# dioph/periodicity

Hardware: AMD Instinct MI355X
Metric: Lomb-Scargle Gpair/s (sample x freq), fp64, N=1e5 x 1e6 per GPU (higher is better)
Workload: dtype f64

## Files before the change

periodicity_amd/_cabi.py:

```python
import ctypes as C
import os
import threading

import numpy as np

_LIB_NAME = "libperiodicity_hip.so"
_lib = None
_lock = threading.Lock()

c_double_p = C.POINTER(C.c_double)
c_int64_p = C.POINTER(C.c_int64)

STATUS_EXC = {-1: ValueError, -2: RuntimeError, -3: RuntimeError, -4: RuntimeError,
              -5: MemoryError}

_VP, _I, _L, _D = C.c_void_p, C.c_int, C.c_int64, C.c_double
PROTOTYPES = {
    "pdc_last_error": (C.c_char_p, []),
    "pdc_version": (_I, []),
    "pdc_device_count": (_I, [C.POINTER(_I)]),
    "pdc_device_info": (_I, [_I, C.c_char_p, _I, C.POINTER(_I), c_int64_p, C.POINTER(_I)]),
    "pdc_release": (_I, []),
    "pdc_alloc_counts": (_I, [c_int64_p, c_int64_p]),
    "pdc_malloc": (_I, [_I, _L, C.POINTER(_VP)]),
# ... 366 lines not shown


def wwz_tile_bins():
    return int(lib().pdc_wwz_tile_bins())


def wwz_work_bytes(n, nf, ntau):
    return int(lib().pdc_wwz_work_bytes(int(n), int(nf), int(ntau)))


def wwz_last_dispatch():
    k, rows, launches = C.c_int(0), C.c_int(0), C.c_int64(0)
    check(lib().pdc_wwz_last_dispatch(C.byref(k), C.byref(rows), C.byref(launches)))
    return k.value, rows.value, launches.value


def bls_scan(t, y, dy, periods, n_bins, len_min, len_max, min_points=5, dips_only=False, slices=0, device=None):
    t, y, periods = _f64(t, "t"), _f64(y, "y"), _f64(periods, "periods")
    dy = None if dy is None else _f64(dy, "dy")
    if y.size != t.size or (dy is not None and dy.size != t.size):
        raise ValueError("Input arrays have incompatible lengths.")
    power, depth = np.empty(periods.size, dtype=np.float64), np.empty(periods.size, dtype=np.float64)
    start, box = np.empty(periods.size, dtype=np.int32), np.empty(periods.size, dtype=np.int32)
    dev = default_device() if device is None else device
    check(lib().pdc_bls_scan(_ptr(t), _ptr(y), _ptr(dy), t.size, _ptr(periods), periods.size, int(n_bins), int(len_min),
                             int(len_max), int(min_points), int(bool(dips_only)), int(slices), _ptr(power), _ptr(depth),
                             _ptr(start), _ptr(box), dev))
    return power, depth, start, box


def gls_scan_batch(t, y, dy, offsets, f0, delta, nf, fit_mean=True, psd=False, shared_t=False,
                   want_power=True, want_peaks=False, j_begin=0, device=None, devices=None):
    t, y = _f64(t, "t"), _f64(y, "y")
    dy = None if dy is None else _f64(dy, "dy")
    offsets = np.ascontiguousarray(offsets, dtype=np.int64)
    nb = offsets.size - 1
    if nb < 1 or offsets[-1] != y.size or (dy is not None and dy.size != y.size):
        raise ValueError("Input arrays have incompatible lengths.")
    if (shared_t and t.size != offsets[1]) or (not shared_t and t.size != y.size):
        raise ValueError("Input arrays have incompatible lengths.")
    power = np.empty((nb, nf), dtype=np.float64) if want_power else None
    amax = np.empty(nb, dtype=np.float64) if want_peaks else None
    argmax = np.empty(nb, dtype=np.int64) if want_peaks else None
    if devices is not None and len(devices) > 1:
        if j_begin:
            raise ValueError("a batch sharded over devices scans the whole grid (j_begin must be 0)")
        devs = np.ascontiguousarray(devices, dtype=np.int32)
        check(lib().pdc_gls_scan_batch_multi(_ptr(t), _ptr(y), _ptr(dy), _ptr(offsets), nb, int(shared_t),
                                             f0, delta, nf, int(bool(fit_mean)), int(bool(psd)),
                                             _ptr(power), _ptr(amax), _ptr(argmax), _ptr(devs), devs.size))
        return power, amax, argmax
    device = pick_device(device, devices)
    dev = default_device() if device is None else device
    check(lib().pdc_gls_scan_batch(_ptr(t), _ptr(y), _ptr(dy), _ptr(offsets), nb, int(shared_t),
                                   f0, delta, j_begin, nf, int(bool(fit_mean)), int(bool(psd)),
                                   _ptr(power), _ptr(amax), _ptr(argmax), dev))
    return power, amax, argmax


def gls_bootstrap(t, y, dy, picks, f0, delta, nf, fit_mean=True, psd=False, method="direct", device=None,
                  devices=None):
    t, y = _f64(t, "t"), _f64(y, "y")
    dy = None if dy is None else _f64(dy, "dy")
    picks = np.ascontiguousarray(picks, dtype=np.int32)
    if y.size != t.size or (dy is not None and dy.size != t.size):
        raise ValueError("Input arrays have incompatible lengths.")
    if picks.ndim != 2 or (picks.shape[0] and picks.shape[1] != t.size):
        raise ValueError("picks must be [n_bootstraps][n_samples]")
    nb = picks.shape[0]
    amax = np.empty(nb, dtype=np.float64)
    argmax = np.empty(nb, dtype=np.int64)
    if devices is not None and len(devices) > 0:
        devs = np.ascontiguousarray(devices, dtype=np.int32)
    else:
        devs = np.array([default_device() if device is None else device], dtype=np.int32)
    check(lib().pdc_gls_bootstrap(_ptr(t), _ptr(y), _ptr(dy), t.size, _ptr(picks), nb, float(f0), float(delta),
                                  int(nf), int(bool(fit_mean)), int(bool(psd)), 1 if method == "fft" else 0,
                                  _ptr(amax), _ptr(argmax), _ptr(devs), devs.size))
    return amax, argmax


GLS_ROUTES = ("none", "general", "parts", "balanced", "shared", "shared2")
_GLS_DISPATCH_FIELDS = ("route", "K", "S", "tiles", "parts", "parts_by_xcd", "bal_slots", "wide_prep", "bpad", "groups",
                        "z_len", "bal_chunks", "lead_swap")


def gls_last_dispatch():
    out = (C.c_int64 * len(_GLS_DISPATCH_FIELDS))()
    check(lib().pdc_test_gls_last_dispatch(out))
    rec = dict(zip(_GLS_DISPATCH_FIELDS, (int(v) for v in out)))
    rec["route"] = GLS_ROUTES[rec["route"]]
    return rec


def gls_last_pair():
    out = (C.c_int64 * 2)()
    check(lib().pdc_test_gls_last_pair(out))
    return bool(out[0]), int(out[1])


def gls_scan_multi(t, y, dy, f0, delta, nf, fit_mean=True, psd=False, devices=(0,)):
    t, y = _f64(t, "t"), _f64(y, "y")
    dy = None if dy is None else _f64(dy, "dy")
    if y.size != t.size or (dy is not None and dy.size != t.size):
        raise ValueError("Input arrays have incompatible lengths.")
    devs = np.ascontiguousarray(devices, dtype=np.int32)
    out = np.empty(nf, dtype=np.float64)
    check(lib().pdc_gls_scan_multi(_ptr(t), _ptr(y), _ptr(dy), t.size, f0, delta, nf,
                                   int(bool(fit_mean)), int(bool(psd)), _ptr(out), _ptr(devs),
                                   devs.size))
    return out


class GlsPlan:

    def __init__(self, devices, n_max, nf_max, loopback_slots=None):
        devs = np.ascontiguousarray(devices, dtype=np.int32)
        self._plan = C.c_void_p()
        if loopback_slots is not None:
            if devs.size != 1:
                raise ValueError("a loopback plan lives on one device")
            self.devices = [int(devs[0])] * int(loopback_slots)
            check(lib().pdc_gls_plan_create_loopback(int(devs[0]), int(loopback_slots), int(n_max),
                                                     int(nf_max), C.byref(self._plan)))
        else:
            self.devices = [int(d) for d in devs]
            check(lib().pdc_gls_plan_create(_ptr(devs), devs.size, int(n_max), int(nf_max),
                                            C.byref(self._plan)))
        self.nf = 0

    def info(self):
        n, r, x = C.c_int(0), C.c_int(0), C.c_int(0)
        check(lib().pdc_gls_plan_info(self._plan, C.byref(n), C.byref(r), C.byref(x)))
        buf = C.create_string_buffer(512)
        check(lib().pdc_gls_plan_init_error(self._plan, buf, 512))
        return {"n_slots": n.value, "rccl_ranks": r.value, "exchange": ("none", "rccl", "copy")[x.value],
                "init_error": buf.value.decode() or None}

    def upload(self, t, y, dy=None):
        t, y = _f64(t, "t"), _f64(y, "y")
        dy = None if dy is None else _f64(dy, "dy")
        if y.size != t.size or (dy is not None and dy.size != t.size):
            raise ValueError("Input arrays have incompatible lengths.")
        check(lib().pdc_gls_plan_upload(self._plan, _ptr(t), _ptr(y), _ptr(dy), t.size))

    def scan(self, f0, delta, nf, fit_mean=True, psd=False):
        check(lib().pdc_gls_plan_scan(self._plan, float(f0), float(delta), int(nf),
                                      int(bool(fit_mean)), int(bool(psd))))
        self.nf = int(nf)

    def wait(self):
        check(lib().pdc_gls_plan_wait(self._plan))

    def download(self, which=0):
        out = np.empty(self.nf, dtype=np.float64)
        check(lib().pdc_gls_plan_download(self._plan, _ptr(out), self.nf, int(which)))
        return out

    def kernel_ms(self):
        ms = C.c_float()
        check(lib().pdc_gls_plan_kernel_ms(self._plan, C.byref(ms)))
        return ms.value

    def slot_ms(self):
        ms = (C.c_float * len(self.devices))()
        check(lib().pdc_gls_plan_slot_ms(self._plan, ms, len(self.devices)))
        return [float(v) for v in ms]
# ... 385 lines not shown
```

periodicity_amd/csrc/gls.hip:

```cpp
#include "pdc_internal.h"
#include "gls_epilogue.h"
#include "gls_sums.h"

#include <cstdlib>

using namespace pdc;

namespace {

constexpr int kBlock = 256;
constexpr int kPrepBlock = 1024;

enum Mode { MODE_FIT_MEAN = 0, MODE_NO_MEAN = 1, MODE_RAW = 2, MODE_TREND = 3 };
constexpr bool mode_fits_mean(int m) { return m == MODE_FIT_MEAN; }
constexpr bool mode_sums_w(int m) { return m == MODE_FIT_MEAN || m == MODE_TREND; }

struct TrendScalars {
    double W;
    double yy, y1, ty, tt, t1;
    double shift;
    double inv_span;
    double prec_a, prec_alpha, prec_beta;
    double log_const;
};

struct GlsArgs {
    const double *rec;
    const int64_t *offsets;
    const double *scal;
    int64_t n_total, n_curves, tiles;
    double f0, delta;
    int64_t j_begin, nf;
    int psd;
    int lead_swap = 0;
    double *power;
    double *raw_s;
    double *raw_c;
    double *blk_max;
    int64_t *blk_arg;
    int64_t z_len = 0;
    int parts = 1, parts_by_xcd = 0;
    double *partial = nullptr;
    int64_t bal_slots = 0, bal_units = 0, bal_chunks = 0, bal_tile_freqs = 0;
    TrendScalars trend = {};
    const double *pair_tab = nullptr;
};

__device__ __forceinline__ int64_t bal_slot_of(const GlsArgs &a, int64_t x) {
    int64_t s = x * a.bal_slots / a.bal_units;
    while ((s + 1) * a.bal_units / a.bal_slots <= x) ++s;
    while (s * a.bal_units / a.bal_slots > x) --s;
    return s;
}

struct PrepArgs {
    const double *t, *y, *dy;
    const int64_t *offsets;
    int64_t n_total;
    int shared_t, fit_mean, raw;
    double delta;
    double *rec, *scal;
    double *rw = nullptr;
    double *tp = nullptr;
    int64_t bpad = 0;
    const int32_t *picks = nullptr;
};

__global__ __launch_bounds__(kPrepBlock) void gls_prep_kernel(PrepArgs a) {
    __shared__ double red[kPrepBlock / 64];
    const int tid = threadIdx.x;
    const int64_t off = a.offsets ? a.offsets[blockIdx.x] : 0;
    const int64_t n = a.offsets ? a.offsets[blockIdx.x + 1] - off : a.n_total;
    const double *t = a.shared_t ? a.t : a.t + off;
    const int32_t *pk = a.picks ? a.picks + off : nullptr;
    const double *y = pk ? a.y : a.y + off;
    const double *dy = a.dy ? (pk ? a.dy : a.dy + off) : nullptr;
    auto at = [pk](int64_t i) -> int64_t { return pk ? (int64_t)pk[i] : i; };
    double *rec = a.rec + off * 6;
    const double t0 = n > 0 ? t[0] : 0.0;

    double W = 1.0, ybar = 0.0;
    if (!a.raw) {
        double acc = 0.0;
        for (int64_t i = tid; i < n; i += kPrepBlock) {
            const double e = dy ? dy[at(i)] : 1.0;
            acc += 1.0 / (e * e);
        }
        W = block_sum<kPrepBlock>(acc, red);
        if (a.fit_mean) {
            acc = 0.0;
            for (int64_t i = tid; i < n; i += kPrepBlock) {
                const double e = dy ? dy[at(i)] : 1.0;
                acc += (1.0 / (e * e)) / W * y[at(i)];
            }
            ybar = block_sum<kPrepBlock>(acc, red);
        }
    }
    double yy = 0.0, wsum = 0.0;
    if (a.rw) {
        for (int64_t i = tid; i < n; i += kPrepBlock) {
            const double e = dy ? dy[at(i)] : 1.0;
            const double w = (1.0 / (e * e)) / W;
            const double yc = y[at(i)] - ybar;
            const double wy = w * yc;
            yy += wy * yc;
            wsum += w;
            if (dy) reinterpret_cast<double2 *>(a.rw)[i * a.bpad + blockIdx.x] = make_double2(wy, w);
            else a.rw[i * a.bpad + blockIdx.x] = wy;
            if (blockIdx.x == 0) a.tp[i] = t[i] - t0;
        }
    } else
    for (int64_t i = tid; i < n; i += kPrepBlock) {
        const double tp = t[i] - t0;
        double w, wy;
        if (a.raw) {
            w = y[at(i)];
            wy = w;
// ... 41 lines not shown
    for (int64_t i = (int64_t)blockIdx.x * kBlock + threadIdx.x; i < a.p.n_total;
         i += (int64_t)gridDim.x * kBlock) {
        const double wr = inv_var(a.p.dy, i);
        sw += wr;
        swy += wr * a.p.y[i];
    }
    sw = block_sum<kBlock>(sw, red);
    swy = block_sum<kBlock>(swy, red);
    if (threadIdx.x == 0) {
        a.part[blockIdx.x] = sw;
        a.part[kPrepParts + blockIdx.x] = swy;
    }
}

__device__ __forceinline__ double fold_partials(const double *p, int count, double *red) {
    double v = 0.0;
    for (int i = threadIdx.x; i < count; i += kBlock) v += p[i];
    return block_sum<kBlock>(v, red);
}

__global__ __launch_bounds__(kBlock) void gls_prep_wide_b(WidePrepArgs a) {
    __shared__ double red[kBlock / 64];
    const double W = fold_partials(a.part, a.nparts, red);
    const double ybar = a.p.fit_mean ? fold_partials(a.part + kPrepParts, a.nparts, red) / W : 0.0;
    const double t0 = a.p.t[0];
    double yy = 0.0, wsum = 0.0;
    for (int64_t i = (int64_t)blockIdx.x * kBlock + threadIdx.x; i < a.p.n_total;
         i += (int64_t)gridDim.x * kBlock) {
        const double tp = a.p.t[i] - t0;
        const double w = inv_var(a.p.dy, i) / W;
        const double yc = a.p.y[i] - ybar;
        const double wy = w * yc;
        yy += wy * yc;
        wsum += w;
        double sd, cd;
        sincos_cycles(frac_product(a.p.delta, tp), sd, cd);
        const double rw = sqrt(w);
        double2 *r = reinterpret_cast<double2 *>(a.p.rec + i * 6);
        r[0] = make_double2(rw * yc, rw);
        r[1] = make_double2(cd, sd);
        r[2] = make_double2(cd + cd, tp);
    }
    yy = block_sum<kBlock>(yy, red);
    wsum = block_sum<kBlock>(wsum, red);
    if (threadIdx.x == 0) {
        a.part[2 * kPrepParts + blockIdx.x] = yy;
        a.part[3 * kPrepParts + blockIdx.x] = wsum;
    }
}

__global__ __launch_bounds__(kBlock) void gls_prep_wide_c(WidePrepArgs a) {
    __shared__ double red[kBlock / 64];
    const double W = fold_partials(a.part, a.nparts, red);
    const double yy = fold_partials(a.part + 2 * kPrepParts, a.nparts, red);
    const double wsum = fold_partials(a.part + 3 * kPrepParts, a.nparts, red);
    if (threadIdx.x == 0) {
        a.p.scal[0] = yy;
        a.p.scal[1] = wsum;
        a.p.scal[2] = W;
        a.p.scal[3] = a.p.t[0];
    }
}

constexpr int kPairM = 8;
constexpr int kPairRow = kPairM * 4;

__global__ __launch_bounds__(kBlock) void gls_pair_table_kernel(const double *rec, double *tab, int64_t n_total, double delta) {
    const int64_t g = (int64_t)blockIdx.x * kBlock + threadIdx.x;
    const int64_t i = g / kPairM;
    if (i >= n_total + 2) return;
    double c = 0.0, s = 0.0, c2 = 0.0, s2 = 0.0;
    if (i < n_total) {
        const double tp = rec[i * 6 + 5];
        const double k = (double)(2 * (int)(g % kPairM) + 1), h = 0.5 * delta;
        const double hi = h * tp, lo = __builtin_fma(h, tp, -hi);
        const double p = k * hi, pe = __builtin_fma(k, hi, -p);
        const double r = (p - __builtin_rint(p)) + __builtin_fma(k, lo, pe);
        sincos_cycles(r, s, c);
        sincos_cycles(r + r, s2, c2);
    }
    double2 *o = reinterpret_cast<double2 *>(tab + g * 4);
    o[0] = make_double2(c, s);
    o[1] = make_double2(c2, s2);
}

template <int MODE>
__device__ __forceinline__ double gls_power(double Sh, double Ch, double S, double C, double SS,
                                            double SC, double YY, double Wsum, double Werr,
                                            int psd) {
    const double S2 = 2.0 * SC;
    const double C2 = Wsum - 2.0 * SS;
    return gls_power_from_sums<mode_fits_mean(MODE)>(Sh, Ch, S, C, S2, C2, YY, Werr, psd);
}

__device__ __forceinline__ double bglst_loglik(double Sh, double Ch, double S, double C, double SS, double SC,
                                               double TS, double TC, double Wsum, const TrendScalars &q) {
    const double tc = TC * q.inv_span + q.shift * C, ts = TS * q.inv_span + q.shift * S;
    const double W = q.W;
    const double m00 = W * (Wsum - SS) + q.prec_a;
    const double m10 = W * SC, m11 = W * SS + q.prec_a;
    const double m20 = W * tc, m21 = W * ts, m22 = W * q.tt + q.prec_alpha;
    const double m30 = W * C, m31 = W * S, m32 = W * q.t1, m33 = W * Wsum + q.prec_beta;
    const double b0 = W * Ch, b1 = W * Sh, b2 = W * q.ty, b3 = W * q.y1;
    const double l00 = __builtin_sqrt(m00);
    const double l10 = m10 / l00, l20 = m20 / l00, l30 = m30 / l00;
    const double l11 = __builtin_sqrt(m11 - l10 * l10);
    const double l21 = (m21 - l20 * l10) / l11, l31 = (m31 - l30 * l10) / l11;
    const double l22 = __builtin_sqrt(m22 - l20 * l20 - l21 * l21);
    const double l32 = (m32 - l30 * l20 - l31 * l21) / l22;
    const double l33 = __builtin_sqrt(m33 - l30 * l30 - l31 * l31 - l32 * l32);
    const double z0 = b0 / l00;
    const double z1 = (b1 - l10 * z0) / l11;
    const double z2 = (b2 - l20 * z0 - l21 * z1) / l22;
    const double z3 = (b3 - l30 * z0 - l31 * z1 - l32 * z2) / l33;
    const double quad = W * q.yy - (z0 * z0 + z1 * z1 + z2 * z2 + z3 * z3);
    const double logdet = 2.0 * (log(l00) + log(l11) + log(l22) + log(l33));
    return -0.5 * (quad + logdet + q.log_const);
}

template <int K, int MODE, int SPLIT, bool BAL = false, bool PAIR = false>
__global__ __launch_bounds__(kBlock, (K >= 16 ? 2 : 1)) void gls_scan_kernel(GlsArgs a) {
    static_assert(!PAIR || (K == 2 * kPairM && (MODE == MODE_FIT_MEAN || MODE == MODE_NO_MEAN)), "mirrored pairs: K = 16, the two GLS modes");
    constexpr int FT = kBlock / SPLIT;
    constexpr bool TIGHT = BAL || K >= 16;
    constexpr int COLS = FT / 64;
    constexpr int kChunk = SPLIT == 1 ? 64 : 128;
    __shared__ double2 tab[kChunk + 1][COLS * 8 + 8 + 1];
    __shared__ double red_v[4];
    __shared__ long long red_i[4];
    __shared__ double2 sc_k[6];
    __shared__ double gf_red[PAIR ? 16 : 1][16];
    __shared__ double gf_acc[16];
    const int tid_ = threadIdx.x;
    if (TIGHT && tid_ < 6) sc_k[tid_] = sincos_coefficient(tid_);

    const int64_t G = BAL ? a.bal_slots : a.n_curves * a.tiles;
    const int64_t per_xcd = (G + 7) / 8;
    int64_t L = (int64_t)(blockIdx.x % 8) * per_xcd + blockIdx.x / 8;
    int zpart = blockIdx.y;
    if (a.parts_by_xcd) {
        const int64_t q = blockIdx.x / 8, zi = q / G;
        L = q - zi * G;
        zpart = (int)(blockIdx.x % 8) + 8 * (int)zi;
        if (zpart >= a.parts) return;
    }
    if (L >= G) return;
    int64_t bal_u = 0, bal_hi = 0;
    if (BAL) {
        bal_u = L * a.bal_units / a.bal_slots;
        bal_hi = (L + 1) * a.bal_units / a.bal_slots;
        if (bal_u >= bal_hi) return;
    }
    do {
    int64_t curve = L / a.tiles;
    int64_t tile = L - curve * a.tiles;
    int64_t bal_take = 0;
    int bal_piece = 0;
    int64_t bal_c0 = 0;
    if (BAL) {
        curve = 0;
        int64_t b_chunks = a.bal_chunks, b_slots = a.bal_slots, b_units = a.bal_units;
        asm volatile("" : "+s"(b_chunks), "+s"(b_slots), "+s"(b_units));
        tile = (bal_hi - 1) / b_chunks;
        const int64_t t0 = tile * b_chunks;
        bal_c0 = (bal_u > t0 ? bal_u : t0) - t0;
        bal_take = bal_hi - t0 - bal_c0;
        int64_t s_of = t0 * b_slots / b_units;
        while ((s_of + 1) * b_units / b_slots <= t0) ++s_of;
        while (s_of * b_units / b_slots > t0) --s_of;
        bal_piece = (int)(L - s_of);
    }

    const int64_t off = a.offsets ? a.offsets[curve] : 0;
    const int64_t n = a.offsets ? a.offsets[curve + 1] - off : a.n_total;
    const int wave = __builtin_amdgcn_readfirstlane(tid_ >> 6), part = wave % SPLIT;
    const int col = wave / SPLIT;
    const int64_t jt = tile * FT * (int64_t)K;
    const int64_t jl = jt + (col * 64 + (tid_ & 63)) * (int64_t)K;
    const double f_tile = __dadd_rn(a.f0, __dmul_rn((double)(a.j_begin + jt), a.delta));
    const double kdelta = (double)K * a.delta;

    static_assert(MODE != MODE_TREND || (SPLIT == 1 && !BAL && K <= 8), "BGLST: eight sums per frequency, whole curves per tile");
    double Sh[K], Ch[K], S[K], C[K], SS[K], SC[K];
    double TS[K], TC[K];
#pragma unroll
    for (int k = 0; k < K; ++k) Sh[k] = Ch[k] = S[k] = C[k] = SS[k] = SC[k] = TS[k] = TC[k] = 0.0;
    if (PAIR) {
        int t16 = tid_;
        asm volatile("" : "+v"(t16));
        if (t16 < 16) gf_acc[t16] = 0.0;
    }

    const int64_t s_begin = BAL ? bal_c0 * kChunk : (a.partial ? (int64_t)zpart * a.z_len : 0);
    const int64_t s_stop = BAL ? s_begin + bal_take * kChunk : s_begin + a.z_len;
    const int64_t s_end = (BAL || a.partial) ? (s_stop < n ? s_stop : n) : n;
    for (int64_t base = s_begin; base < s_end; base += kChunk) {
        __syncthreads();
        int tid = tid_;
        if (TIGHT) asm volatile("" : "+v"(tid));
        const int lane = tid & 63;
        const int slot_a = col * 8 + (lane >> 3), slot_b = COLS * 8 + (lane & 7);
        if (PAIR) {
            constexpr int SPP = kChunk / 16;
            const int m16 = tid & 15, seg = tid >> 4;
            const int64_t i0 = base + seg * SPP;
            const double *tp_ = a.pair_tab + (off + i0) * kPairRow + (m16 & 7) * 4 + (m16 < 8 ? 1 : 3);
            const double *rp_ = a.rec + (off + i0) * 6 + 1;
            double acc = 0.0;
#pragma unroll
            for (int q = 0; q < SPP; ++q) {
                const bool live = i0 + q < s_end;
                const double sq = live ? rp_[q * 6] : 0.0;
                const double v = live ? tp_[q * kPairRow] : 0.0;
                acc = __builtin_fma(sq * sq, m16 < 8 ? v * v : v, acc);
            }
            gf_red[seg][m16] = acc;
            __builtin_amdgcn_sched_barrier(0);
        }
        if (tid < 2 * kChunk) {
            const int il = tid >> 1;
            const bool live = base + il < s_end;
            const double tp = live ? a.rec[(off + base + il) * 6 + 5] : 0.0;
            const double sqw = live ? a.rec[(off + base + il) * 6 + 1] : 0.0;
            double2 step1, cur;
            double2 kk[6];
            if (TIGHT) {
#pragma unroll
                for (int q = 0; q < 6; ++q) kk[q] = sc_k[q];
            }
            auto sincos_fill = [&](const double r, double &s_, double &c_) {
                if (TIGHT) sincos_cycles_k(r, kk, s_, c_);
                else sincos_cycles(r, s_, c_);
            };
            if ((tid & 1) == 0) {
                sincos_fill(frac_product(kdelta, tp), step1.x, step1.y);
                double one = 1.0, zero = 0.0;
                if (TIGHT) asm volatile("" : "+v"(one), "+v"(zero));
                tab[il][COLS * 8] = make_double2(zero, one);
                tab[il][COLS * 8 + 1] = step1;
                cur = step1;
#pragma unroll
                for (int q = 2; q < 8; ++q) {
                    cur = rot2(cur, step1);
                    tab[il][COLS * 8 + q] = cur;
                }
                double r_base = frac_product(f_tile, tp);
                if (PAIR) {
                    double dl = a.delta;
                    asm volatile("" : "+v"(dl));
                    r_base += frac_product(8.0 * dl, tp) - frac_product(0.5 * dl, tp);
                }
                sincos_fill(r_base, cur.x, cur.y);
                if (MODE == MODE_FIT_MEAN || MODE == MODE_NO_MEAN || MODE == MODE_TREND) {
                    cur.x *= sqw;
                    cur.y *= sqw;
                }
            } else {
                sincos_fill(frac_product(8.0 * kdelta, tp), step1.x, step1.y);
            }
            double2 b0;
            b0.x = __shfl_xor(cur.x, 1, 64);
            b0.y = __shfl_xor(cur.y, 1, 64);
            if (tid & 1) {
                tab[il][0] = b0;
#pragma unroll
                for (int q = 1; q < COLS * 8; ++q) {
                    b0 = rot2(b0, step1);
                    tab[il][q] = b0;
                }
            }
        }
        __syncthreads();
        const int cnt = (int)((s_end - base) < kChunk ? (s_end - base) : kChunk);
        const int i_end = cnt < (part + 1) * (kChunk / SPLIT) ? cnt : (part + 1) * (kChunk / SPLIT);
        const int i_beg = part * (kChunk / SPLIT);
        if constexpr (PAIR) {
            if (tid < 16) {
                double g = gf_red[0][tid];
#pragma unroll
                for (int q = 1; q < 16; ++q) g += gf_red[q][tid];
                gf_acc[tid] += g;
            }
            using d8 = double __attribute__((ext_vector_type(8)));
            using cd8 = __attribute__((address_space(4))) const d8;
            using d2 = double __attribute__((ext_vector_type(2)));
            using cd2 = __attribute__((address_space(4))) const d2;
            auto uniform = [](const double *p) {
                const uintptr_t u = reinterpret_cast<uintptr_t>(p);
                const uint32_t lo_ = __builtin_amdgcn_readfirstlane((uint32_t)u), hi_ = __builtin_amdgcn_readfirstlane((uint32_t)(u >> 32));
                return ((uintptr_t)hi_ << 32) | lo_;
            };
            const cd8 *stab = reinterpret_cast<const cd8 *>(uniform(a.pair_tab + (off + base) * kPairRow));
            const cd2 *srec = reinterpret_cast<const cd2 *>(uniform(a.rec + (off + base) * 6));
            const int i_last = __builtin_amdgcn_readfirstlane(i_end);
            d8 fa, fb, ga, gb;
            d2 r;
            double2 qa, qt;
#ifdef PDC_GLS_PROBE_ROW0
            auto trow = [](const int) { return 0; };
#else
            auto trow = [](const int i) { return i * 4; };
#endif
            const int q0 = COLS >= 2 ? (a.lead_swap & col & 1) * 2 : 0;
            const cd8 *stab_f = stab + q0, *stab_g = stab + (2 - q0);
            auto request_first = [&](const int i) {
                fa = stab_f[trow(i)];
                fb = stab_f[trow(i) + 1];
                r = srec[i * 3];
                qa = tab[i][slot_a];
                qt = tab[i][slot_b];
            };
            double A1, B1, A2, B2, a2, ab;
            auto pair_fmas = [&](const d8 &h, const int m0) {
#pragma unroll
                for (int q = 0; q < 2; ++q) {
                    const int hi = K / 2 + m0 + q, lo = K / 2 - 1 - m0 - q;
                    const double c = h[4 * q], s = h[4 * q + 1], c2 = h[4 * q + 2], s2 = h[4 * q + 3];
                    Sh[hi] = __builtin_fma(c, A1, Sh[hi]);
                    Sh[lo] = __builtin_fma(s, B1, Sh[lo]);
                    Ch[hi] = __builtin_fma(c, B1, Ch[hi]);
                    Ch[lo] = __builtin_fma(s, A1, Ch[lo]);
                    if (mode_sums_w(MODE)) {
                        S[hi] = __builtin_fma(c, A2, S[hi]);
                        S[lo] = __builtin_fma(s, B2, S[lo]);
                        C[hi] = __builtin_fma(c, B2, C[hi]);
                        C[lo] = __builtin_fma(s, A2, C[lo]);
                    }
                    SS[hi] = __builtin_fma(c2, a2, SS[hi]);
                    SS[lo] = __builtin_fma(s2, ab, SS[lo]);
                    SC[hi] = __builtin_fma(c2, ab, SC[hi]);
                    SC[lo] = __builtin_fma(s2, a2, SC[lo]);
                }
            };
            if (i_beg < i_last) {
                request_first(i_beg);
                for (int i = i_beg; i < i_last; ++i) {
                    __builtin_amdgcn_s_waitcnt(0xc07f);
                    ga = stab_g[trow(i)];
                    gb = stab_g[trow(i) + 1];
                    __builtin_amdgcn_sched_barrier(0);
                    const double2 seed = rot2(qa, qt);
                    A1 = r[0] * seed.x;
                    B1 = r[0] * seed.y;
                    A2 = r[1] * seed.x;
                    B2 = r[1] * seed.y;
                    a2 = seed.x * seed.x;
                    ab = seed.x * seed.y;
                    pair_fmas(fa, 0);
                    pair_fmas(fb, 2);
                    __builtin_amdgcn_sched_barrier(0);
                    __builtin_amdgcn_s_waitcnt(0xc07f);
                    request_first(i + 1);
                    __builtin_amdgcn_sched_barrier(0);
                    pair_fmas(ga, 4);
                    pair_fmas(gb, 6);
                    __builtin_amdgcn_sched_barrier(0);
                }
            }
        } else {
        using d4 = double __attribute__((ext_vector_type(4)));
// ... 616 lines not shown

void tile_shape(int64_t n_curves, int64_t nf, int64_t n_total, bool may_split, int *K_out, int *S_out, int *Z_out) {
    static const int envK = [] { const char *e = getenv("PDC_GLS_K"); return e ? atoi(e) : 0; }();
    static const int envS = [] { const char *e = getenv("PDC_GLS_S"); return e ? atoi(e) : 0; }();
    static const int envZ = [] { const char *e = getenv("PDC_GLS_Z"); return e ? atoi(e) : 0; }();
    int64_t z_max = 1;
    if (may_split && n_curves == 1 && n_total >= 16384) {
        z_max = n_total / 2048;
        const int64_t room = kPartialCells / (nf > 0 ? nf : 1);
        z_max = z_max < room ? z_max : room;
        z_max = z_max > kPartsMax ? kPartsMax : (z_max < 1 ? 1 : z_max);
    }
    double best = 1e300;
    int bk = 8, bs = 1, bz = 1;
    for (int K : {16, 8, 4}) {
        if (envK && K != envK) continue;
        for (int S : {1, 2, 4}) {
            if (envS && S != envS) continue;
            const double tile_waves = (double)n_curves * (double)((nf + 64 * K - 1) / (64 * K)) * S;
            int64_t Z = (int64_t)__builtin_ceil(2048.0 / tile_waves);
            Z = Z > z_max ? z_max : (Z < 1 ? 1 : Z);
            if (Z >= 8) Z -= Z % 8;
            if (envZ) Z = envZ > z_max ? z_max : envZ;
            const double waves = tile_waves * (double)Z;
            const double rounds = __builtin_ceil(waves / 1024.0);
            double cost = rounds * (12.0 + 8.0 * K) / ((double)S * (double)Z);
            if (waves / 1024.0 <= 1.0) cost *= 1.10;
            cost *= 1.0 + 0.02 * (S > 2 ? S - 2 : 2 - S);
            if (Z > 1) cost *= 1.02;
            if (cost < best) {
                best = cost;
                bk = K;
                bs = S;
                bz = (int)Z;
            }
        }
    }
    *K_out = bk;
    *S_out = bs;
    *Z_out = bz;
}

template <int MODE, int S>
void launch_scan_ks(int K, dim3 grid, hipStream_t st, const GlsArgs &a) {
    if constexpr (MODE == MODE_FIT_MEAN || MODE == MODE_NO_MEAN) {
        if (K == 16 && a.pair_tab) {
            hipLaunchKernelGGL((gls_scan_kernel<16, MODE, S, false, true>), grid, dim3(kBlock), 0, st, a);
            return;
        }
    }
    switch (K) {
        case 4: hipLaunchKernelGGL((gls_scan_kernel<4, MODE, S>), grid, dim3(kBlock), 0, st, a); break;
        case 16: hipLaunchKernelGGL((gls_scan_kernel<16, MODE, S>), grid, dim3(kBlock), 0, st, a); break;
        default: hipLaunchKernelGGL((gls_scan_kernel<8, MODE, S>), grid, dim3(kBlock), 0, st, a); break;
    }
}

template <int MODE>
void launch_scan_balanced(int S, dim3 grid, hipStream_t st, const GlsArgs &a) {
    if (a.pair_tab) {
        if (S == 2) hipLaunchKernelGGL((gls_scan_kernel<16, MODE, 2, true, true>), grid, dim3(kBlock), 0, st, a);
        else hipLaunchKernelGGL((gls_scan_kernel<16, MODE, 4, true, true>), grid, dim3(kBlock), 0, st, a);
    } else {
        if (S == 2) hipLaunchKernelGGL((gls_scan_kernel<16, MODE, 2, true>), grid, dim3(kBlock), 0, st, a);
        else hipLaunchKernelGGL((gls_scan_kernel<16, MODE, 4, true>), grid, dim3(kBlock), 0, st, a);
    }
}

template <int MODE>
void launch_scan(int K, int S, dim3 grid, hipStream_t st, const GlsArgs &a) {
    switch (S) {
        case 4: launch_scan_ks<MODE, 4>(K, grid, st, a); break;
        case 2: launch_scan_ks<MODE, 2>(K, grid, st, a); break;
        default: launch_scan_ks<MODE, 1>(K, grid, st, a); break;
    }
}

struct WorkLayout {
    int64_t rec, scal, parts, blk_max, blk_arg, partial, pair, total;
};

enum Route { ROUTE_NONE = 0, ROUTE_GENERAL = 1, ROUTE_PARTS = 2, ROUTE_BALANCED = 3, ROUTE_SHARED = 4, ROUTE_SHARED2 = 5 };
struct Dispatch {
    int64_t route, K, S, tiles, parts, parts_by_xcd, bal_slots, wide_prep, bpad, groups, z_len, bal_chunks, lead_swap;
};
thread_local Dispatch g_last_dispatch = {};
struct PairUse {
    int64_t ran, table_bytes;
};
thread_local PairUse g_last_pair = {};

WorkLayout layout(int64_t n_total, int64_t n_curves, int64_t nf) {
    auto up = [](int64_t x) { return (x + 255) & ~(int64_t)255; };
    const int64_t tiles_max = (nf + 63) / 64;
    WorkLayout w;
    w.rec = 0;
    w.scal = up(n_total * 48);
    w.parts = w.scal + up(n_curves * 32);
    w.blk_max = w.parts + up(4 * kPrepParts * 8);
    w.blk_arg = w.blk_max + up(n_curves * tiles_max * 8);
    w.partial = w.blk_arg + up(n_curves * tiles_max * 8);
    int64_t cells = kPartsMax * nf < kPartialCells ? kPartsMax * nf : kPartialCells;
    cells = cells > 3 * nf ? cells : 3 * nf;
    w.pair = w.partial + (n_curves == 1 ? up(cells * 6 * 8) : 0);
    w.total = w.pair + up((n_total + 2) * kPairRow * 8);
    return w;
}

int scan_dev(int device, hipStream_t st, const double *d_t, const double *d_y, const double *d_dy,
             const int64_t *d_offsets, int64_t n_total, int64_t n_curves, int shared_t, double f0,
             double delta, int64_t j_begin, int64_t nf, int mode, int psd, double *d_power,
             double *d_raw_s, double *d_raw_c, double *d_amax, int64_t *d_argmax, void *work,
             int64_t work_bytes, const int32_t *d_picks = nullptr, const TrendScalars *trend = nullptr) {
    PDC_REQUIRE(d_t && d_y, "gls: t and y must not be NULL");
    PDC_REQUIRE((mode == MODE_TREND) == (trend != nullptr) && (mode != MODE_TREND || (n_curves == 1 && !d_picks && !shared_t)),
                "gls: the trend mode takes one curve and its scalars");
    PDC_REQUIRE(!d_picks || (shared_t && d_offsets && mode != MODE_RAW), "gls: picks need a shared time axis");
    PDC_REQUIRE(n_total >= 0 && n_curves >= 1 && nf >= 0 && j_begin >= 0, "gls: negative size");
    PDC_REQUIRE(n_curves == 1 || d_offsets, "gls: a batch needs offsets");
    PDC_REQUIRE(n_curves * ((nf + 255) / 256 + 1) < (int64_t)1 << 31, "gls: grid too large");
    const WorkLayout w = layout(n_total, n_curves, nf);
    PDC_REQUIRE(work && work_bytes >= w.total, "gls: workspace too small (%lld < %lld bytes)",
                (long long)work_bytes, (long long)w.total);
    if (nf == 0) return PDC_OK;
    PDC_TRY(use_device(device));
    char *base = static_cast<char *>(work);
    Dispatch &rec = g_last_dispatch;
    rec = Dispatch{};
    rec.parts = 1;
    g_last_pair = PairUse{};

    PrepArgs p;
    p.t = d_t;
    p.y = d_y;
    p.dy = d_dy;
    p.offsets = d_offsets;
    p.n_total = n_total;
    p.shared_t = shared_t;
    p.fit_mean = mode == MODE_FIT_MEAN;
    p.raw = mode == MODE_RAW;
    p.delta = delta;
    p.rec = reinterpret_cast<double *>(base + w.rec);
    p.scal = reinterpret_cast<double *>(base + w.scal);
    p.picks = d_picks;
    const bool peaks = d_amax || d_argmax;

    static const int env_shared = [] { const char *e = getenv("PDC_GLS_SHARED"); return e ? atoi(e) : -1; }();
    if (shared_t && mode != MODE_RAW && n_curves >= 2 && env_shared != 0) {
        const bool uni = d_dy == nullptr;
        const int64_t n = n_total / n_curves;
        const int64_t group = (int64_t)kShWaves * (uni ? kShCurvesU : kShCurvesW);
        const int64_t bpad = (n_curves + group - 1) / group * group;
        const int64_t table = (n + 2) * bpad * (uni ? 8 : 16);
        if ((n_curves >= 96 || env_shared == 1) && table + n * 8 <= w.scal && n * n_curves == n_total) {
            p.rw = p.rec;
            p.tp = reinterpret_cast<double *>(base + table);
            p.bpad = bpad;
            PDC_HIP(hipMemsetAsync(base + table / (n + 2) * n, 0, table / (n + 2) * 2, st));
            hipLaunchKernelGGL(gls_prep_kernel, dim3((unsigned)n_curves), dim3(kPrepBlock), 0, st, p);
            PDC_HIP(hipGetLastError());
            SharedArgs sa;
            sa.tp = p.tp;
            sa.rw = p.rw;
            sa.scal = p.scal;
            sa.n = n;
            sa.n_curves = n_curves;
            sa.bpad = bpad;
            sa.tiles = (nf + 63) / 64;
            sa.groups = bpad / group;
            sa.f0 = f0;
            sa.delta = delta;
            sa.j_begin = j_begin;
            sa.nf = nf;
            sa.psd = psd;
            sa.power = d_power;
            sa.blk_max = peaks ? reinterpret_cast<double *>(base + w.blk_max) : nullptr;
            sa.blk_arg = peaks ? reinterpret_cast<int64_t *>(base + w.blk_arg) : nullptr;
            static const bool sh2 = [] { const char *e = getenv("PDC_GLS_SH2"); return !(e && e[0] == '0'); }();
            if (!uni && sh2) {
                sa.groups = bpad / (kSh2Waves * kSh2Curves);
                const int64_t G2 = sa.groups * ((nf + 127) / 128);
                PDC_REQUIRE(G2 < (int64_t)1 << 31, "gls: grid too large");
                const dim3 grid2((unsigned)(((G2 + 7) / 8) * 8));
                rec.route = ROUTE_SHARED2;
                rec.K = 2;
                rec.tiles = (nf + 127) / 128;
                rec.bpad = bpad;
                rec.groups = sa.groups;
                if (mode == MODE_FIT_MEAN) {
                    PDC_TRY(allow_dynamic_lds((const void *)gls_shared2_kernel<true>, (int)kSh2Lds));
                    hipLaunchKernelGGL((gls_shared2_kernel<true>), grid2, dim3(kSh2Block), kSh2Lds, st, sa);
                } else {
                    PDC_TRY(allow_dynamic_lds((const void *)gls_shared2_kernel<false>, (int)kSh2Lds));
                    hipLaunchKernelGGL((gls_shared2_kernel<false>), grid2, dim3(kSh2Block), kSh2Lds, st, sa);
                }
                PDC_HIP(hipGetLastError());
                if (peaks) {
                    hipLaunchKernelGGL(gls_peak_kernel, dim3((unsigned)n_curves), dim3(64), 0, st, sa.blk_max,
                                       sa.blk_arg, sa.tiles, d_amax, d_argmax);
                    PDC_HIP(hipGetLastError());
                }
                return PDC_OK;
            }
            const int64_t G = sa.groups * sa.tiles;
            PDC_REQUIRE(G < (int64_t)1 << 31, "gls: grid too large");
            const dim3 grid((unsigned)(((G + 7) / 8) * 8));
            rec.route = ROUTE_SHARED;
            rec.K = 1;
            rec.tiles = sa.tiles;
            rec.bpad = bpad;
            rec.groups = sa.groups;
            if (mode == MODE_FIT_MEAN) {
                if (uni) hipLaunchKernelGGL((gls_shared_kernel<true, true>), grid, dim3(kShBlock), 0, st, sa);
                else hipLaunchKernelGGL((gls_shared_kernel<true, false>), grid, dim3(kShBlock), 0, st, sa);
            } else {
                if (uni) hipLaunchKernelGGL((gls_shared_kernel<false, true>), grid, dim3(kShBlock), 0, st, sa);
                else hipLaunchKernelGGL((gls_shared_kernel<false, false>), grid, dim3(kShBlock), 0, st, sa);
            }
            PDC_HIP(hipGetLastError());
            if (peaks) {
                hipLaunchKernelGGL(gls_peak_kernel, dim3((unsigned)n_curves), dim3(64), 0, st, sa.blk_max,
                                   sa.blk_arg, sa.tiles, d_amax, d_argmax);
                PDC_HIP(hipGetLastError());
            }
            return PDC_OK;
        }
    }
    if (n_curves == 1 && mode != MODE_RAW && n_total >= 16384 && !d_picks) {
        WidePrepArgs wp;
        wp.p = p;
        wp.nparts = (int)((n_total + 4 * kBlock - 1) / (4 * kBlock));
        wp.nparts = wp.nparts > kPrepParts ? kPrepParts : wp.nparts;
        wp.part = reinterpret_cast<double *>(base + w.parts);
        rec.wide_prep = 1;
        hipLaunchKernelGGL(gls_prep_wide_a, dim3(wp.nparts), dim3(kBlock), 0, st, wp);
        hipLaunchKernelGGL(gls_prep_wide_b, dim3(wp.nparts), dim3(kBlock), 0, st, wp);
        hipLaunchKernelGGL(gls_prep_wide_c, dim3(1), dim3(kBlock), 0, st, wp);
    } else {
        hipLaunchKernelGGL(gls_prep_kernel, dim3((unsigned)n_curves), dim3(kPrepBlock), 0, st, p);
    }
    PDC_HIP(hipGetLastError());

    int K, S, parts;
    tile_shape(n_curves, nf, n_total, mode != MODE_RAW, &K, &S, &parts);
    if (mode == MODE_TREND) {
        K = K > 8 ? 8 : K;
        S = 1;
        parts = 1;
    }
    GlsArgs a;
    if (trend) a.trend = *trend;
    a.rec = p.rec;
    a.offsets = d_offsets;
    a.scal = p.scal;
    a.n_total = n_total;
    a.n_curves = n_curves;
    static const int env_pair = [] { const char *e = getenv("PDC_GLS_PAIR"); return e ? atoi(e) : -1; }();
    if (K == 16 && (mode == MODE_FIT_MEAN || mode == MODE_NO_MEAN) && env_pair != 0) {
        double *tab = reinterpret_cast<double *>(base + w.pair);
        const int64_t cells = (n_total + 2) * kPairM;
        PDC_REQUIRE((cells + kBlock - 1) / kBlock < (int64_t)1 << 31, "gls: too many samples for the offset table");
        hipLaunchKernelGGL(gls_pair_table_kernel, dim3((unsigned)((cells + kBlock - 1) / kBlock)), dim3(kBlock), 0, st,
                           (const double *)p.rec, tab, n_total, delta);
        PDC_HIP(hipGetLastError());
        a.pair_tab = tab;
        static const int env_lead = [] { const char *e = getenv("PDC_GLS_LEAD"); return e ? atoi(e) : 0; }();
        a.lead_swap = (env_lead == 1 && S <= 2) ? 1 : 0;
        rec.lead_swap = a.lead_swap;
        g_last_pair.ran = 1;
        g_last_pair.table_bytes = (n_total + 2) * kPairRow * 8;
    }
    const int64_t tile_freqs = (int64_t)(kBlock / S) * K;
    a.tiles = (nf + tile_freqs - 1) / tile_freqs;
    a.f0 = f0;
    a.delta = delta;
    a.j_begin = j_begin;
    a.nf = nf;
    a.psd = psd;
    a.power = d_power;
    a.raw_s = d_raw_s;
    a.raw_c = d_raw_c;
    a.blk_max = peaks ? reinterpret_cast<double *>(base + w.blk_max) : nullptr;
    a.blk_arg = peaks ? reinterpret_cast<int64_t *>(base + w.blk_arg) : nullptr;
    const int64_t G = a.n_curves * a.tiles;
    dim3 grid((unsigned)(((G + 7) / 8) * 8));
    if (parts > 1) {
        const int64_t chunk = 128;
        a.z_len = ((n_total + parts - 1) / parts + chunk - 1) / chunk * chunk;
        parts = (int)((n_total + a.z_len - 1) / a.z_len);
        a.partial = reinterpret_cast<double *>(base + w.partial);
        a.parts = parts;
        if (parts >= 8) {
            a.parts_by_xcd = 1;
            grid.x = (unsigned)(8 * ((parts + 7) / 8) * G);
        } else {
            grid.y = (unsigned)parts;
        }
    }
    rec.route = parts > 1 ? ROUTE_PARTS : ROUTE_GENERAL;
    rec.K = K;
    rec.S = S;
    rec.tiles = a.tiles;
    rec.parts = parts;
    rec.parts_by_xcd = a.parts_by_xcd;
    rec.z_len = a.z_len;
    static const int env_bal = [] { const char *e = getenv("PDC_GLS_BAL"); return e ? atoi(e) : -1; }();
    bool balanced = false;
    if (n_curves == 1 && parts == 1 && mode != MODE_RAW && mode != MODE_TREND && K == 16 && S >= 2 && env_bal != 0) {
        const int64_t slots = 512, nchunks = (n_total + 127) / 128;
        const int64_t full = a.tiles / slots, rem = a.tiles % slots;
        const double t_tiles = (double)full + (rem == 0 ? 0.0 : (rem <= slots / 2 ? 0.5 : 1.0));
        const double t_bal = (double)a.tiles / (double)slots + 0.004;
        const int64_t w_bal = (a.tiles + slots - 1) / slots * slots;
        if ((env_bal == 1 || t_tiles > 1.02 * t_bal) && a.tiles * 2 > w_bal && nchunks >= 32) {
            balanced = true;
            a.bal_slots = w_bal;
            a.bal_chunks = nchunks;
            a.bal_units = a.tiles * nchunks;
            a.bal_tile_freqs = tile_freqs;
            a.partial = reinterpret_cast<double *>(base + w.partial);
            grid = dim3((unsigned)(((w_bal + 7) / 8) * 8));
            rec.route = ROUTE_BALANCED;
            rec.bal_slots = w_bal;
            rec.bal_chunks = nchunks;
            if (mode == MODE_FIT_MEAN) launch_scan_balanced<MODE_FIT_MEAN>(S, grid, st, a);
            else launch_scan_balanced<MODE_NO_MEAN>(S, grid, st, a);
        }
    }
    if (balanced) {
    } else if (mode == MODE_TREND) {
        if (K == 4) hipLaunchKernelGGL((gls_scan_kernel<4, MODE_TREND, 1>), grid, dim3(kBlock), 0, st, a);
        else hipLaunchKernelGGL((gls_scan_kernel<8, MODE_TREND, 1>), grid, dim3(kBlock), 0, st, a);
    } else if (mode == MODE_FIT_MEAN) {
        launch_scan<MODE_FIT_MEAN>(K, S, grid, st, a);
    } else if (mode == MODE_NO_MEAN) {
        launch_scan<MODE_NO_MEAN>(K, S, grid, st, a);
    } else {
        launch_scan<MODE_RAW>(K, S, grid, st, a);
    }
    PDC_HIP(hipGetLastError());
    int64_t peak_tiles = a.tiles;
    if (a.partial) {
        peak_tiles = (nf + kBlock / 4 - 1) / (kBlock / 4);
        if (mode == MODE_FIT_MEAN)
            hipLaunchKernelGGL(gls_finish_kernel<MODE_FIT_MEAN>, dim3((unsigned)peak_tiles), dim3(kBlock), 0, st, a, parts);
        else
            hipLaunchKernelGGL(gls_finish_kernel<MODE_NO_MEAN>, dim3((unsigned)peak_tiles), dim3(kBlock), 0, st, a, parts);
        PDC_HIP(hipGetLastError());
    }
    if (peaks) {
        hipLaunchKernelGGL(gls_peak_kernel, dim3((unsigned)n_curves), dim3(64), 0, st, a.blk_max,
                           a.blk_arg, peak_tiles, d_amax, d_argmax);
        PDC_HIP(hipGetLastError());
    }
    return PDC_OK;
}

}

extern "C" {

int pdc_test_gls_last_dispatch(int64_t *out) {
    PDC_REQUIRE(out, "pdc_test_gls_last_dispatch: NULL argument");
    const Dispatch &d = g_last_dispatch;
    const int64_t v[13] = {d.route, d.K, d.S, d.tiles, d.parts, d.parts_by_xcd, d.bal_slots, d.wide_prep,
                           d.bpad, d.groups, d.z_len, d.bal_chunks, d.lead_swap};
    for (int i = 0; i < 13; ++i) out[i] = v[i];
    return PDC_OK;
}

int pdc_test_gls_last_pair(int64_t *out) {
    PDC_REQUIRE(out, "pdc_test_gls_last_pair: NULL argument");
    out[0] = g_last_pair.ran;
    out[1] = g_last_pair.table_bytes;
    return PDC_OK;
}

int64_t pdc_gls_work_bytes(int64_t n_total, int64_t n_curves, int64_t nf) {
    if (n_total < 0 || n_curves < 1 || nf < 0) return -1;
    return layout(n_total, n_curves, nf).total;
}

int pdc_gls_scan_dev(int device, void *stream, const double *d_t, const double *d_y,
                     const double *d_dy, const int64_t *d_offsets, int64_t n_total,
                     int64_t n_curves, int shared_t, double f0, double delta, int64_t j_begin,
                     int64_t nf, int fit_mean, int psd, double *d_power, double *d_amax,
                     int64_t *d_argmax, void *work, int64_t work_bytes) {
    PDC_REQUIRE(d_power || d_amax || d_argmax, "gls: no output requested");
    return scan_dev(device, (hipStream_t)stream, d_t, d_y, d_dy, d_offsets, n_total, n_curves,
                    shared_t, f0, delta, j_begin, nf, fit_mean ? MODE_FIT_MEAN : MODE_NO_MEAN, psd,
                    d_power, nullptr, nullptr, d_amax, d_argmax, work, work_bytes);
}

namespace {
__global__ void gls_iota_offsets_kernel(int64_t *offsets, int64_t n, int64_t count) {
    const int64_t b = (int64_t)blockIdx.x * blockDim.x + threadIdx.x;
    if (b <= count) offsets[b] = b * n;
}
}

int64_t pdc_gls_bootstrap_work_bytes(int64_t n, int64_t n_boot, int64_t nf) {
    if (n < 0 || n_boot < 1 || nf < 0) return -1;
    return layout(n * n_boot, n_boot, nf).total + (((n_boot + 1) * 8 + 255) & ~(int64_t)255);
}

int pdc_gls_bootstrap_dev(int device, void *stream, const double *d_t, const double *d_y, const double *d_dy,
                          int64_t n, const int32_t *d_picks, int64_t n_boot, double f0, double delta, int64_t nf,
                          int fit_mean, int psd, double *d_amax, int64_t *d_argmax, void *work,
                          int64_t work_bytes) {
    PDC_REQUIRE(d_t && d_y && d_picks && (d_amax || d_argmax), "gls_bootstrap: NULL argument");
    PDC_REQUIRE(n >= 0 && n < ((int64_t)1 << 31) && n_boot >= 1 && nf >= 0, "gls_bootstrap: bad size");
    const int64_t need = pdc_gls_bootstrap_work_bytes(n, n_boot, nf);
    PDC_REQUIRE(work && work_bytes >= need, "gls_bootstrap: workspace too small (%lld < %lld bytes)",
                (long long)work_bytes, (long long)need);
    if (nf == 0) return PDC_OK;
    PDC_TRY(use_device(device));
    const int64_t inner = layout(n * n_boot, n_boot, nf).total;
    int64_t *d_off = reinterpret_cast<int64_t *>(static_cast<char *>(work) + inner);
    hipLaunchKernelGGL(gls_iota_offsets_kernel, dim3((unsigned)((n_boot + 256) / 256)), dim3(256), 0,
                       (hipStream_t)stream, d_off, n, n_boot);
    PDC_HIP(hipGetLastError());
    return scan_dev(device, (hipStream_t)stream, d_t, d_y, d_dy, d_off, n * n_boot, n_boot, 1, f0, delta, 0, nf,
                    fit_mean ? MODE_FIT_MEAN : MODE_NO_MEAN, psd, nullptr, nullptr, nullptr, d_amax, d_argmax, work,
                    inner, d_picks);
}

int pdc_gls_scan_batch(const double *t, const double *y, const double *dy, const int64_t *offsets,
                       int64_t n_curves, int shared_t, double f0, double delta, int64_t j_begin,
                       int64_t nf, int fit_mean, int psd, double *power_out, double *amax_out,
                       int64_t *argmax_out, int device) {
    PDC_REQUIRE(t && y && offsets, "gls: t, y and offsets must not be NULL");
    PDC_REQUIRE(n_curves >= 1 && nf >= 0 && j_begin >= 0, "gls: negative size");
    PDC_REQUIRE(power_out || amax_out || argmax_out, "gls: no output requested");
    GlsBatchIn in;
    PDC_TRY(in.check("gls", offsets, n_curves, shared_t));
    HostCall hc(device);
    const int64_t wb = pdc_gls_work_bytes(in.n_total, n_curves, nf);
    in.upload(hc, t, y, dy, offsets, n_curves);
    double *d_pow = power_out ? hc.out<double>(SLOT_OUT0, n_curves * nf * 8) : nullptr;
    double *d_amax = amax_out ? hc.out<double>(SLOT_OUT1, n_curves * 8) : nullptr;
    int64_t *d_arg = argmax_out ? hc.out<int64_t>(SLOT_OUT2, n_curves * 8) : nullptr;
    void *d_work = hc.reserve(SLOT_WORK, wb);
    PDC_TRY(hc.status);
    PDC_TRY(scan_dev(device, hc.stream(), in.d_t, in.d_y, in.d_dy, in.d_off, in.n_total, n_curves, shared_t, f0, delta,
                     j_begin, nf, fit_mean ? MODE_FIT_MEAN : MODE_NO_MEAN, psd, d_pow, nullptr, nullptr, d_amax, d_arg,
                     d_work, wb));
    hc.back(power_out, d_pow, n_curves * nf * 8);
    hc.back(amax_out, d_amax, n_curves * 8);
    hc.back(argmax_out, d_arg, n_curves * 8);
    return hc.finish();
// ... 61 lines not shown
```

Baseline: 4198.

## Precompute per-chunk pair sums and per-sample step rotations for GLS pair path

Adds a prepass kernel that computes per-sample step sincos values, and a second kernel that reduces per-chunk pair-table sums once, ahead of the scan. In the pair path the scan kernel then reads these stored values instead of recomputing the chunk sums in every tile. The fill is split so one set of threads builds the base column by rotation while another builds the step columns. This removes per-tile redundant reductions and a sincos call, at the cost of extra workspace, more prepass launches and rotation-accumulated rounding.

```diff
diff --git a/periodicity_amd/_cabi.py b/periodicity_amd/_cabi.py
--- a/periodicity_amd/_cabi.py
+++ b/periodicity_amd/_cabi.py
@@ -472,7 +472,7 @@
 
 GLS_ROUTES = ("none", "general", "parts", "balanced", "shared", "shared2")
 _GLS_DISPATCH_FIELDS = ("route", "K", "S", "tiles", "parts", "parts_by_xcd", "bal_slots", "wide_prep", "bpad", "groups",
-                        "z_len", "bal_chunks", "lead_swap")
+                        "z_len", "bal_chunks", "lead_swap", "chunk_sums")
 
 
 def gls_last_dispatch():
diff --git a/periodicity_amd/csrc/gls.hip b/periodicity_amd/csrc/gls.hip
--- a/periodicity_amd/csrc/gls.hip
+++ b/periodicity_amd/csrc/gls.hip
@@ -32,7 +32,7 @@
     double f0, delta;
     int64_t j_begin, nf;
     int psd;
-    int lead_swap = 0;
+    int16_t lead_swap = 0, chunk_sums = 0;
     double *power;
     double *raw_s;
     double *raw_c;
@@ -240,6 +240,71 @@
     double2 *o = reinterpret_cast<double2 *>(tab + g * 4);
     o[0] = make_double2(c, s);
     o[1] = make_double2(c2, s2);
+}
+
+constexpr int kPairStep = 4;
+__host__ __device__ constexpr int64_t pair_chunk_rows(int64_t n_total, int64_t n_curves, int chunk) { return n_total / chunk + n_curves; }
+__host__ __device__ __forceinline__ const double *pair_step(const double *tab, int64_t n_total) { return tab + (n_total + 2) * kPairRow; }
+__host__ __device__ __forceinline__ const double *pair_chunk_sums(const double *tab, int64_t n_total) {
+    return pair_step(tab, n_total) + n_total * kPairStep;
+}
+
+__global__ __launch_bounds__(kBlock) void gls_pair_step_kernel(const double *rec, double *step, int64_t n_total, double delta) {
+    const int64_t i = (int64_t)blockIdx.x * kBlock + threadIdx.x;
+    if (i >= n_total) return;
+    double2 kk[6];
+#pragma unroll
+    for (int q = 0; q < 6; ++q) kk[q] = sincos_coefficient(q);
+    const double tp = rec[i * 6 + 5];
+    const double kdelta = 16.0 * delta;
+    double2 s1, s8;
+    sincos_cycles_k(frac_product(kdelta, tp), kk, s1.x, s1.y);
+    sincos_cycles_k(frac_product(8.0 * kdelta, tp), kk, s8.x, s8.y);
+    double2 *o = reinterpret_cast<double2 *>(step + i * kPairStep);
+    o[0] = s1;
+    o[1] = s8;
+}
+
+template <int CHUNK>
+__global__ __launch_bounds__(kBlock) void gls_pair_chunk_kernel(const double *rec, const double *tab, const int64_t *offsets,
+                                                                int64_t n_total, int64_t n_curves, double *sums) {
+    __shared__ double red[16][16];
+    const int tid = threadIdx.x;
+    const int64_t row = blockIdx.x;
+    int64_t c = 0;
+    if (offsets) {
+        int64_t hi = n_curves - 1;
+        while (c < hi) {
+            const int64_t mid = (c + hi + 1) / 2;
+            if (offsets[mid] / CHUNK + mid <= row) c = mid;
+            else hi = mid - 1;
+        }
+    }
+    const int64_t off = offsets ? offsets[c] : 0;
+    const int64_t n = offsets ? offsets[c + 1] - off : n_total;
+    const int64_t base = (row - (off / CHUNK + c)) * CHUNK;
+    if (base >= n) return;
+    constexpr int SPP = CHUNK / 16;
+    const int m16 = tid & 15, seg = tid >> 4;
+    const int64_t i0 = base + seg * SPP;
+    const double *tp_ = tab + (off + i0) * kPairRow + (m16 & 7) * 4 + (m16 < 8 ? 1 : 3);
+    const double *rp_ = rec + (off + i0) * 6 + 1;
+    double acc = 0.0;
+#pragma unroll
+    for (int q = 0; q < SPP; ++q) {
+        const bool live = i0 + q < n;
+        const double sq = live ? rp_[q * 6] : 0.0;
+        const double v = live ? tp_[q * kPairRow] : 0.0;
+        acc = __builtin_fma(sq * sq, m16 < 8 ? v * v : v, acc);
+    }
+    red[seg][m16] = acc;
+    __syncthreads();
+    if (tid < 16) {
+        double g = red[0][tid];
+#pragma unroll
+        for (int q = 1; q < 16; ++q) g += red[q][tid];
+        sums[row * 16 + tid] = g;
+    }
 }
 
 template <int MODE>
@@ -358,23 +423,83 @@
         if (TIGHT) asm volatile("" : "+v"(tid));
         const int lane = tid & 63;
         const int slot_a = col * 8 + (lane >> 3), slot_b = COLS * 8 + (lane & 7);
-        if (PAIR) {
-            constexpr int SPP = kChunk / 16;
-            const int m16 = tid & 15, seg = tid >> 4;
-            const int64_t i0 = base + seg * SPP;
-            const double *tp_ = a.pair_tab + (off + i0) * kPairRow + (m16 & 7) * 4 + (m16 < 8 ? 1 : 3);
-            const double *rp_ = a.rec + (off + i0) * 6 + 1;
-            double acc = 0.0;
-#pragma unroll
-            for (int q = 0; q < SPP; ++q) {
-                const bool live = i0 + q < s_end;
-                const double sq = live ? rp_[q * 6] : 0.0;
-                const double v = live ? tp_[q * kPairRow] : 0.0;
-                acc = __builtin_fma(sq * sq, m16 < 8 ? v * v : v, acc);
-            }
-            gf_red[seg][m16] = acc;
-            __builtin_amdgcn_sched_barrier(0);
-        }
+        if constexpr (PAIR) {
+#ifdef PDC_GLS_PROBE_FILL
+            const bool fill_now = base == s_begin;
+#else
+            constexpr bool fill_now = true;
+#endif
+            const bool stored = a.chunk_sums != 0;
+            if (!stored && fill_now) {
+                constexpr int SPP = kChunk / 16;
+                const int m16 = tid & 15, seg = tid >> 4;
+                const int64_t i0 = base + seg * SPP;
+                const double *tp_ = a.pair_tab + (off + i0) * kPairRow + (m16 & 7) * 4 + (m16 < 8 ? 1 : 3);
+                const double *rp_ = a.rec + (off + i0) * 6 + 1;
+                double acc = 0.0;
+#pragma unroll
+                for (int q = 0; q < SPP; ++q) {
+                    const bool live = i0 + q < s_end;
+                    const double sq = live ? rp_[q * 6] : 0.0;
+                    const double v = live ? tp_[q * kPairRow] : 0.0;
+                    acc = __builtin_fma(sq * sq, m16 < 8 ? v * v : v, acc);
+                }
+                gf_red[seg][m16] = acc;
+                __builtin_amdgcn_sched_barrier(0);
+            }
+            const int il = tid & (kChunk - 1);
+            const bool live = base + il < s_end;
+            const double2 *stp = reinterpret_cast<const double2 *>(pair_step(a.pair_tab, a.n_total) + (off + base + il) * kPairStep);
+            if (tid < kChunk) {
+                if (fill_now) {
+                    const double tp = live ? a.rec[(off + base + il) * 6 + 5] : 0.0;
+                    const double sqw = live ? a.rec[(off + base + il) * 6 + 1] : 0.0;
+                    const double2 step8 = live ? stp[1] : make_double2(0.0, 0.0);
+                    double2 kk[6];
+#pragma unroll
+                    for (int q = 0; q < 6; ++q) kk[q] = sc_k[q];
+                    double r_base = frac_product(f_tile, tp);
+                    double dl = a.delta;
+                    asm volatile("" : "+v"(dl));
+                    r_base += frac_product(8.0 * dl, tp) - frac_product(0.5 * dl, tp);
+                    double2 b0;
+                    sincos_cycles_k(r_base, kk, b0.x, b0.y);
+                    b0.x *= sqw;
+                    b0.y *= sqw;
+                    tab[il][0] = b0;
+#pragma unroll
+                    for (int q = 1; q < COLS * 8; ++q) {
+                        b0 = rot2(b0, step8);
+                        tab[il][q] = b0;
+                    }
+                }
+            } else if (tid < 2 * kChunk) {
+                double touch0 = 0.0, touch1 = 0.0;
+                if (stored && live) {
+                    const double *row = a.pair_tab + (off + base + il) * kPairRow;
+                    touch0 = row[0];
+                    touch1 = row[kPairRow / 2];
+                }
+                if (fill_now) {
+                    double g_chunk = 0.0;
+                    if (stored && il < 16)
+                        g_chunk = pair_chunk_sums(a.pair_tab, a.n_total)[(off / kChunk + curve + base / kChunk) * 16 + il];
+                    const double2 step1 = live ? stp[0] : make_double2(0.0, 0.0);
+                    double one = 1.0, zero = 0.0;
+                    asm volatile("" : "+v"(one), "+v"(zero));
+                    tab[il][COLS * 8] = make_double2(zero, one);
+                    tab[il][COLS * 8 + 1] = step1;
+                    double2 cur = step1;
+#pragma unroll
+                    for (int q = 2; q < 8; ++q) {
+                        cur = rot2(cur, step1);
+                        tab[il][COLS * 8 + q] = cur;
+                    }
+                    if (stored && il < 16) gf_acc[il] += g_chunk;
+                }
+                asm volatile("" : : "v"(touch0), "v"(touch1));
+            }
+        } else {
         if (tid < 2 * kChunk) {
             const int il = tid >> 1;
             const bool live = base + il < s_end;
@@ -402,13 +527,7 @@
                     cur = rot2(cur, step1);
                     tab[il][COLS * 8 + q] = cur;
                 }
-                double r_base = frac_product(f_tile, tp);
-                if (PAIR) {
-                    double dl = a.delta;
-                    asm volatile("" : "+v"(dl));
-                    r_base += frac_product(8.0 * dl, tp) - frac_product(0.5 * dl, tp);
-                }
-                sincos_fill(r_base, cur.x, cur.y);
+                sincos_fill(frac_product(f_tile, tp), cur.x, cur.y);
                 if (MODE == MODE_FIT_MEAN || MODE == MODE_NO_MEAN || MODE == MODE_TREND) {
                     cur.x *= sqw;
                     cur.y *= sqw;
@@ -428,12 +547,17 @@
                 }
             }
         }
+        }
         __syncthreads();
         const int cnt = (int)((s_end - base) < kChunk ? (s_end - base) : kChunk);
         const int i_end = cnt < (part + 1) * (kChunk / SPLIT) ? cnt : (part + 1) * (kChunk / SPLIT);
         const int i_beg = part * (kChunk / SPLIT);
         if constexpr (PAIR) {
-            if (tid < 16) {
+#ifdef PDC_GLS_PROBE_FILL
+            if (tid < 16 && !a.chunk_sums && base == s_begin) {
+#else
+            if (tid < 16 && !a.chunk_sums) {
+#endif
                 double g = gf_red[0][tid];
 #pragma unroll
                 for (int q = 1; q < 16; ++q) g += gf_red[q][tid];
@@ -1216,7 +1340,7 @@
 
 enum Route { ROUTE_NONE = 0, ROUTE_GENERAL = 1, ROUTE_PARTS = 2, ROUTE_BALANCED = 3, ROUTE_SHARED = 4, ROUTE_SHARED2 = 5 };
 struct Dispatch {
-    int64_t route, K, S, tiles, parts, parts_by_xcd, bal_slots, wide_prep, bpad, groups, z_len, bal_chunks, lead_swap;
+    int64_t route, K, S, tiles, parts, parts_by_xcd, bal_slots, wide_prep, bpad, groups, z_len, bal_chunks, lead_swap, chunk_sums;
 };
 thread_local Dispatch g_last_dispatch = {};
 struct PairUse {
@@ -1237,7 +1361,7 @@
     int64_t cells = kPartsMax * nf < kPartialCells ? kPartsMax * nf : kPartialCells;
     cells = cells > 3 * nf ? cells : 3 * nf;
     w.pair = w.partial + (n_curves == 1 ? up(cells * 6 * 8) : 0);
-    w.total = w.pair + up((n_total + 2) * kPairRow * 8);
+    w.total = w.pair + up(((n_total + 2) * kPairRow + n_total * kPairStep + pair_chunk_rows(n_total, n_curves, 64) * 16) * 8);
     return w;
 }
 
@@ -1397,6 +1521,11 @@
         hipLaunchKernelGGL(gls_pair_table_kernel, dim3((unsigned)((cells + kBlock - 1) / kBlock)), dim3(kBlock), 0, st,
                            (const double *)p.rec, tab, n_total, delta);
         PDC_HIP(hipGetLastError());
+        if (n_total > 0) {
+            hipLaunchKernelGGL(gls_pair_step_kernel, dim3((unsigned)((n_total + kBlock - 1) / kBlock)), dim3(kBlock), 0, st,
+                               (const double *)p.rec, const_cast<double *>(pair_step(tab, n_total)), n_total, delta);
+            PDC_HIP(hipGetLastError());
+        }
         a.pair_tab = tab;
         static const int env_lead = [] { const char *e = getenv("PDC_GLS_LEAD"); return e ? atoi(e) : 0; }();
         a.lead_swap = (env_lead == 1 && S <= 2) ? 1 : 0;
@@ -1431,6 +1560,16 @@
             grid.y = (unsigned)parts;
         }
     }
+    static const int env_chunk = [] { const char *e = getenv("PDC_GLS_CHUNK_SUMS"); return e ? atoi(e) : 1; }();
+    if (a.pair_tab && n_total > 0 && env_chunk != 0 && (parts == 1 || a.z_len % (S == 1 ? 64 : 128) == 0)) {
+        double *sums = const_cast<double *>(pair_chunk_sums(a.pair_tab, n_total));
+        const dim3 rows((unsigned)pair_chunk_rows(n_total, n_curves, S == 1 ? 64 : 128));
+        if (S == 1) hipLaunchKernelGGL(gls_pair_chunk_kernel<64>, rows, dim3(kBlock), 0, st, a.rec, a.pair_tab, d_offsets, n_total, n_curves, sums);
+        else hipLaunchKernelGGL(gls_pair_chunk_kernel<128>, rows, dim3(kBlock), 0, st, a.rec, a.pair_tab, d_offsets, n_total, n_curves, sums);
+        PDC_HIP(hipGetLastError());
+        a.chunk_sums = 1;
+    }
+    rec.chunk_sums = a.chunk_sums;
     rec.route = parts > 1 ? ROUTE_PARTS : ROUTE_GENERAL;
     rec.K = K;
     rec.S = S;
@@ -1497,9 +1636,9 @@
 int pdc_test_gls_last_dispatch(int64_t *out) {
     PDC_REQUIRE(out, "pdc_test_gls_last_dispatch: NULL argument");
     const Dispatch &d = g_last_dispatch;
-    const int64_t v[13] = {d.route, d.K, d.S, d.tiles, d.parts, d.parts_by_xcd, d.bal_slots, d.wide_prep,
-                           d.bpad, d.groups, d.z_len, d.bal_chunks, d.lead_swap};
-    for (int i = 0; i < 13; ++i) out[i] = v[i];
+    const int64_t v[14] = {d.route, d.K, d.S, d.tiles, d.parts, d.parts_by_xcd, d.bal_slots, d.wide_prep,
+                           d.bpad, d.groups, d.z_len, d.bal_chunks, d.lead_swap, d.chunk_sums};
+    for (int i = 0; i < 14; ++i) out[i] = v[i];
     return PDC_OK;
 }
 
```

Result: faster. 4268 (median of 6 runs) (+1.7%).
